# CobaltCrabby/ray_tracer

Measured on AMD Instinct MI355X. Metric: Mrays/s (reference-semantics closest-hit queries) at 1920x1080 Sponza, higher is better.
Workload: dtype f32; 1 GPU; sponza (synthetic-262267-tris), 1920x1080, 8 spp/step, bounceLimit 8, rows interleaved over 1 GPU(s), up to 10 steps in flight per rank (groups of 10+9+9+9); scene=sponza, assets=synthetic-262267-tris, width=1920, height=1080, frames_in_flight=10, pipeline=multi-kernel (k_trace_pw + k_shade per round)

## Files before the change

ray_tracer_amd/csrc/rt_device.hip:

```cpp

#include "rt_kernels.hip.h"
#include "bvh_build.hip.h"

#include <dlfcn.h>
#include <rccl/rccl.h>

#include <algorithm>
#include <chrono>
#include <cmath>
#include <cstdio>
#include <cstdlib>
#include <string>
#include <type_traits>
#include <vector>

namespace {

struct DevBuf {
    void* p = nullptr;
    size_t bytes = 0;
    DevBuf() = default;
    DevBuf(DevBuf&& o) noexcept : p(o.p), bytes(o.bytes) { o.p = nullptr; o.bytes = 0; }
    ~DevBuf() { release(); }
    void release() { if (p) (void)hipFree(p); p = nullptr; bytes = 0; }
};

struct EventPair { hipEvent_t a, b; };
#define RT_MAX_LANES 4
#define RT_FRAMES_MAX_SLOTS (24ull << 20)
struct RootInfo { uint32_t idx, cnt; float lo[3], hi[3]; uint32_t triFirst, triTotal; };
struct RowsOf {
    uint32_t width = 0, height = 0, row0 = 0, rowStride = 0, nRows = 0;
    bool whole(uint32_t w, uint32_t h) const { return width == w && height == h && row0 == 0 && rowStride == 1 && nRows == h; }
};

}

struct rt_ctx {
    std::string error;
    int device = 0, numCUs = 256;
    hipStream_t ownStream = nullptr, stream = nullptr;
    DevScene sc{};
    std::vector<DevBuf> sceneBufs;
    DevBuf texelBuf, texInfoBuf, triUVBuf, objTreeBuf, objCostBuf;
    DevBuf matBuf, sphereBuf, sphereMatBuf, objInvBuf, objFwdBuf, objMetaBuf, objBoxBuf, objSkipBuf, maskBoxBuf, emitBuf, emitPreBuf;
    std::vector<RayMaterial> hostMats;
    std::vector<uint32_t> hostSphereMat, hostObjMat, hostObjRoot, hostObjSampler;
    DevBuf objAlphaBuf;
    uint32_t maxLeafDepth = 0;
    std::vector<uint32_t> nodeRemap;
    std::vector<RootInfo> rootOf;
    bool cull = false;
    ncclComm_t comm = nullptr;
    int commRanks = 0, commRank = 0;
    DevBuf gatherBuf;
    DevBuf stateBuf, queueBuf, fbBuf, counterBuf, scratchBuf;
    DevBuf overflowBuf[RT_MAX_LANES];
    hipStream_t sideStream[RT_MAX_LANES - 1] = {};
    hipEvent_t forkEvent = nullptr, joinEvent[RT_MAX_LANES - 1] = {}, pollEventSide[RT_MAX_LANES - 1] = {};
    uint32_t capacity = 0;
    PathState ps{}; Queues q{};
    uint32_t* hostCounts = nullptr;
    uint32_t fbPixels = 0; bool fbValid = false;
    bool profiling = false;
    std::vector<EventPair> evPool;
    size_t evUsed = 0;
    hipEvent_t profBase = nullptr;
    DevCounters* snap = nullptr;
    hipEvent_t snapEvent = nullptr;
    hipEvent_t pollEvent = nullptr;
    DevBuf probeBuf;
    DevBuf waveTimeBuf;
    DevBuf aovBuf, aovCounterBuf;
    DevBuf shadeStatBuf;
    uint32_t aovPixels = 0; bool aovValid = false;
    RowsOf fbRows, aovRows;
    DevBuf dnWorkBuf, dnHostBuf, dnOutBuf;
    size_t dnOutPixels = 0; bool dnValid = false;

    struct Tuning {
        int objTreeMin = 48;
        int framesPerLaunch = 0;
        uint64_t framesMaxSlots = RT_FRAMES_MAX_SLOTS;
        int cameraReuse = 1;
        int lightQueries = 1;
        int lanes = 3;
        bool lanesSet = false;
        uint32_t lanesMinSlots = 1u << 20;
        int laneGridPct = 0;
        int traceVariant = 1;
        int pipeline = -1;
        uint32_t fusedBelowPixels = 4000000;
        uint32_t fusedBelowBoxTests = 70;
        int refill = 8;
        int refillMk = 16;
        bool refillMkSet = false;
        int chunk = 256;
        int ldsStackCap = 24;
        int fastLanes = 32;
        bool fastLanesSet = false;
        int wSetup = 16, wLeaf = 16;
        bool wSetupSet = false, wLeafSet = false;
        int wSetupFused = 16, wLeafFused = 24;
        int blocksPerCU = 0;
        int phaseStats = 0;
        int tileSlots = 1;
        int fastShare = 10;
        int maskIdentity = 0;
        int scatter = -1;
        int hotPairs = 2;
        int pixelRefill = 0;
        int batchPixels = 0;
        int batchFixed = 80;
        int fusedMaps = 0;
        int probe = 1;
    } tune;

    struct Measured {
        bool snapPending = false;
        unsigned long long snapBox = 0, snapRays = 0, snapSeg = 0, snapPaths = 0;
        double boxPerRay = -1.0;
        double segPerPath = -1.0;
    } meas;

    struct Reports {
        int lastPipeline = 0;
        int lastParts = 1;
        char lastKernel[96] = "";
        size_t waveTimesCount = 0;
        double traceMs = 0.0;
        uint64_t traceLaunches = 0;
        std::vector<std::pair<float, float>> traceSpans;
        uint64_t traceLaunchesTotal = 0, aovLaunches = 0;
        double bvhBuildMs = 0.0;
    } rep;
    int fail(const std::string& m) { error = m; return -1; }
    int hip(hipError_t e, const char* what) {
        if (e == hipSuccess) return 0;
        error = std::string(what) + ": " + hipGetErrorString(e);
        return -(int)e - 1000;
    }
};

#define RT_HIP(ctx, call)                                    \
    do {                                                     \
        int _rc = (ctx)->hip((call), #call);                 \
        if (_rc) return _rc;                                 \
    } while (0)

namespace {

int dev_alloc(rt_ctx* c, DevBuf& b, size_t bytes) {
    if (b.p && b.bytes >= bytes) return 0;
    b.release();
    if (bytes == 0) bytes = 256;
    RT_HIP(c, hipMalloc(&b.p, bytes));
    b.bytes = bytes;
    return 0;
}

int upload(rt_ctx* c, DevBuf& b, const void* src, size_t bytes) {
    int rc = dev_alloc(c, b, bytes);
    if (rc) return rc;
    if (bytes) RT_HIP(c, hipMemcpyAsync(b.p, src, bytes, hipMemcpyHostToDevice, c->stream));
    RT_HIP(c, hipStreamSynchronize(c->stream));
    return 0;
}

void pack_materials(const RayMaterial* m, uint32_t n, std::vector<float4>& out) {
    out.resize((size_t)std::max(n, 1u) * 3);
    for (uint32_t i = 0; i < n; i++) {
        out[3 * i + 0] = make_float4(m[i].albedo[0], m[i].albedo[1], m[i].albedo[2], m[i].reflectance);
// ... 793 lines not shown
    if ((rc = upload(c, c->sceneBufs[1], tpos.data(), tpos.size() * sizeof(float4)))) return rc;
    if ((rc = upload(c, c->sceneBufs[2], tnrm.data(), tnrm.size() * sizeof(float4)))) return rc;
    c->sc.nodes = (const float4*)c->sceneBufs[0].p;
    c->sc.triPos = (const float4*)c->sceneBufs[1].p;
    c->sc.triNrm = (const float4*)c->sceneBufs[2].p;
    if ((rc = upload(c, c->sceneBufs[3], leafFirst.data(), leafFirst.size() * 4))) return rc;
    c->sc.leafFirst = (const uint32_t*)c->sceneBufs[3].p;
    if ((rc = upload(c, c->sceneBufs[4], nodesPk.data(), nodesPk.size() * sizeof(float4)))) return rc;
    c->sc.nodesPk = (const float4*)c->sceneBufs[4].p;
    c->sc.nodeCount = devCount;
    c->sc.triCount = nTris;

    if (s->materialCount == 0) return c->fail("scene needs at least one material");
    if ((rc = rt_update_materials(c, s->materials, s->materialCount))) return rc;
    for (uint32_t i = 0; i < s->sphereCount; i++)
        if (s->spheres[i].materialIndex >= s->materialCount) return c->fail("sphere.materialIndex out of range");
    if ((rc = rt_update_spheres(c, s->spheres, s->sphereCount))) return rc;
    return rt_update_objects(c, s->objects, s->objectCount);
}

int rt_sync(rt_ctx* c) {
    if (!c) return -1;
    RT_HIP(c, hipStreamSynchronize(c->stream));
    return harvest_events(c);
}

}

namespace {
int check_tile(rt_ctx* c, const PushConstants* pc, uint32_t width, uint32_t height, uint32_t row0, uint32_t rowStride, uint32_t nRows,
               const char* fn) {
    if (width == 0 || height == 0 || rowStride == 0) return c->fail(std::string(fn) + ": bad image geometry");
    if (nRows && (uint64_t)row0 + (uint64_t)(nRows - 1) * rowStride >= height) return c->fail(std::string(fn) + ": rows exceed the image");
    if (!c->sc.nodes) return c->fail(std::string(fn) + " before rt_upload_scene");
    const RayTracerData& td = pc->rayTraceParams;
    if (td.sphereCount > c->sc.sphereCount) return c->fail("rayTraceParams.sphereCount exceeds the uploaded spheres");
    if (td.objectCount > c->sc.objectCount) return c->fail("rayTraceParams.objectCount exceeds the uploaded objects");
    return 0;
}

DevScene dispatch_scene(const rt_ctx* c, const RayTracerData& td) {
    DevScene sc = c->sc;
    sc.sphereCount = td.sphereCount;
    sc.objectCount = td.objectCount;
    if (sc.objectCount < c->sc.objectCount) { sc.reachCount = 0; sc.objTreeLevels = 0; }
    return sc;
}

FrameParams frame_camera(const rt_ctx* c, const PushConstants* pc, uint32_t width, uint32_t height, uint32_t row0, uint32_t rowStride,
                         uint32_t nRows, uint32_t nPixels) {
    FrameParams fp{};
    memcpy(fp.camRot, pc->camInfo.cameraRotation, 64);
    memcpy(fp.camPos, pc->camInfo.pos, 12);
    fp.planeHeight = pc->camInfo.nearPlane * rt_tan(rt_radians(pc->camInfo.fov * 0.5f)) * 2.f;
    fp.planeWidth = fp.planeHeight * pc->camInfo.aspectRatio;
    fp.bottomLeft[0] = -fp.planeWidth / 2.f;
    fp.bottomLeft[1] = -fp.planeHeight / 2.f;
    fp.bottomLeft[2] = 0.1f;
    fp.tiled = (c->tune.tileSlots && (width % 8u) == 0u) ? 1u : 0u;
    fp.width = width; fp.height = height; fp.row0 = row0; fp.rowStride = rowStride; fp.nRows = nRows; fp.nPixels = nPixels;
    return fp;
}

int choose_pipeline(const rt_ctx::Tuning& t, int pipeline, double boxPerRay, const DevScene& sc, uint32_t nSlots) {
    const bool shortRays = boxPerRay >= 0.0 && boxPerRay < (double)t.fusedBelowBoxTests;
    double sizeLimit = (double)t.fusedBelowPixels;
    if (boxPerRay > 90.0) sizeLimit = std::max(0.375 * sizeLimit, sizeLimit - (boxPerRay - 90.0) * (0.625 / 60.0) * sizeLimit);
    const bool bigScene = (uint64_t)sc.nodeCount * 32u + (uint64_t)sc.triCount * 48u > (4ull << 20);
    const bool shortButMissing = shortRays && bigScene && boxPerRay >= 25.0 && nSlots >= (10u << 20);
    const int chosen = pipeline >= 0 ? pipeline : (((double)nSlots < sizeLimit || (shortRays && !shortButMissing)) ? 1 : 0);
    return (sc.mapFlags && !t.fusedMaps) ? 0 : chosen;
}

int choose_parts(const rt_ctx::Tuning& t, const Dispatch& d, bool cull, double boxPerRay, uint32_t samples, uint32_t nSlots) {
    int nLanes = (samples > 0 && nSlots >= t.lanesMinSlots) ? std::max(1, std::min(t.lanes, (int)RT_MAX_LANES)) : 1;
    if (d.phaseStats) nLanes = 1;
    if (!t.lanesSet && cull && boxPerRay >= 150.0 && nSlots >= (8u << 20)) nLanes = 1;
    return nLanes;
}
int part_grid_pct(const rt_ctx::Tuning& t, int nLanes, uint32_t firstPartSlots) {
    return nLanes > 1 ? (t.laneGridPct > 0 ? t.laneGridPct : (firstPartSlots < 1200000u ? 40 : 50)) : 100;
}

int ensure_part_streams(rt_ctx* c, int nLanes) {
    for (int l = 1; l < nLanes; l++) {
        if (!c->sideStream[l - 1]) {
            if (hipStreamCreateWithFlags(&c->sideStream[l - 1], hipStreamNonBlocking) != hipSuccess) { c->sideStream[l - 1] = nullptr; nLanes = l; break; }
            if (hipEventCreateWithFlags(&c->joinEvent[l - 1], hipEventDisableTiming) != hipSuccess ||
                hipEventCreateWithFlags(&c->pollEventSide[l - 1], hipEventDisableTiming) != hipSuccess) { nLanes = l; break; }
        }
    }
    if (nLanes > 1 && !c->forkEvent && hipEventCreateWithFlags(&c->forkEvent, hipEventDisableTiming) != hipSuccess) { c->forkEvent = nullptr; nLanes = 1; }
    return nLanes;
}

struct Lane { Dispatch d; hipEvent_t poll; uint32_t begin, n, ubActive; int cur; bool pollPending, done; };
void slice_parts(rt_ctx* c, const Dispatch& d, uint32_t nSlots, uint32_t nFrames, int nLanes, Lane* lane) {
    const uint32_t unit = 256u * std::max(1u, nFrames);
    const uint32_t units = (nSlots + unit - 1) / unit;
    uint32_t at = 0;
    for (int l = 0; l < nLanes; l++) {
        const uint32_t u = units / (uint32_t)nLanes + ((uint32_t)l < units % (uint32_t)nLanes ? 1u : 0u);
        const uint32_t end = std::min(nSlots, at + u * unit);
        lane[l] = Lane{d, l ? c->pollEventSide[l - 1] : c->pollEvent, at, end - at, end - at, 0, false, end == at};
        lane[l].d.stream = l ? c->sideStream[l - 1] : c->stream; lane[l].d.counts = c->q.counts + 16 * l; lane[l].d.part = l;
        at = end;
    }
    const int gridPct = part_grid_pct(c->tune, nLanes, lane[0].n);
    for (int l = 0; l < nLanes; l++) lane[l].d.gridPct = gridPct;
}

int render_rounds(rt_ctx* c, const FrameParams& fp, Lane* lane, int nLanes) {
    DevCounters* dc = (DevCounters*)c->counterBuf.p;
    int rc = 0;
    if (nLanes > 1) {
        RT_HIP(c, hipEventRecord(c->forkEvent, c->stream));
        for (int l = 1; l < nLanes; l++) RT_HIP(c, hipStreamWaitEvent(lane[l].d.stream, c->forkEvent, 0));
    }
    const uint64_t maxRounds = (uint64_t)fp.samples * ((uint64_t)fp.bounceLimit + 1);
    for (uint64_t it = 0; it < maxRounds; it++) {
        bool any = false;
        for (int l = 0; l < nLanes; l++) {
            Lane& L = lane[l];
            if (L.done) continue;
            any = true;
            const hipStream_t stream = L.d.stream; uint32_t* const counts = L.d.counts;
            const int cur = L.cur, nxt = cur ^ 1;
            uint32_t* const active[2] = {c->q.active[0] + L.begin, c->q.active[1] + L.begin};
            uint32_t* const rays[2] = {c->q.rays[0] + 3 * (size_t)L.begin, c->q.rays[1] + 3 * (size_t)L.begin};
            hipLaunchKernelGGL(k_zero_counts, dim3(1), dim3(64), 0, stream, counts + nxt, counts + 2 + nxt, counts + 4, counts + 5 + nxt, counts + 7 + nxt);
            TraceArgs ta{rays[cur], counts + 2 + cur, nullptr, nullptr, dc, counts + 5 + cur, counts + 7 + cur, L.n};
            const uint64_t ubRays = std::min<uint64_t>((uint64_t)L.ubActive * 3, (uint64_t)L.n * 3);
            if ((rc = launch_trace(c, L.d, (uint32_t)ubRays, ta))) break;
            ShadeArgs sa{active[cur], counts + cur, active[nxt], rays[nxt], counts + nxt, counts + 2 + nxt, (ShadeStatStripe*)c->shadeStatBuf.p, counts + 5 + nxt, counts + 7 + nxt, L.n};
            if (L.d.sc.mapFlags & (RT_MAP_METALNESS | RT_MAP_BUMP)) hipLaunchKernelGGL(k_shade_maps, dim3((L.ubActive + RT_BLOCK - 1) / RT_BLOCK), dim3(RT_BLOCK), 0, stream, L.d.sc, c->ps, sa, fp);
            else hipLaunchKernelGGL(k_shade, dim3((L.ubActive + RT_BLOCK - 1) / RT_BLOCK), dim3(RT_BLOCK), 0, stream, L.d.sc, c->ps, sa, fp);
            L.cur = nxt;
            if (L.pollPending && hipEventQuery(L.poll) == hipSuccess) {
                L.pollPending = false;
                L.ubActive = std::min(L.ubActive, c->hostCounts[8 + l]);
                if (L.ubActive == 0) { L.done = true; continue; }
            }
            if (!L.pollPending && (it & 7u) == 7u) {
                if (hipMemcpyAsync(c->hostCounts + 8 + l, counts + L.cur, 4, hipMemcpyDeviceToHost, stream) == hipSuccess &&
                    hipEventRecord(L.poll, stream) == hipSuccess)
                    L.pollPending = true;
            }
        }
        if (!any || rc) break;
    }
    for (int l = 1; l < nLanes; l++) {
        RT_HIP(c, hipEventRecord(c->joinEvent[l - 1], lane[l].d.stream));
        RT_HIP(c, hipStreamWaitEvent(c->stream, c->joinEvent[l - 1], 0));
    }
    hipLaunchKernelGGL(k_fold_shade_stats, dim3(1), dim3(RT_STAT_STRIPES), 0, c->stream, (ShadeStatStripe*)c->shadeStatBuf.p, dc);
    return rc;
}

int render_parts(rt_ctx* c, const FrameParams& fp, const Dispatch& d, uint32_t nSlots, float4* fb) {
    const int nLanes = ensure_part_streams(c, choose_parts(c->tune, d, c->cull, c->meas.boxPerRay, fp.samples, nSlots));
    c->rep.lastParts = nLanes;
    Lane lane[RT_MAX_LANES];
    slice_parts(c, d, nSlots, fp.nFrames, nLanes, lane);
    for (int l = 0; l < nLanes; l++) {
        const Lane& L = lane[l];
        if (!L.n) continue;
        hipLaunchKernelGGL(k_raygen, dim3((L.n + RT_BLOCK - 1) / RT_BLOCK), dim3(RT_BLOCK), 0, c->stream, d.sc, c->ps,
                           c->q.active[0] + L.begin, c->q.rays[0] + 3 * (size_t)L.begin, fp, L.begin, L.begin + L.n);
        if (fp.samples > 0) hipLaunchKernelGGL(k_init_counts, dim3(1), dim3(64), 0, c->stream, L.d.counts, L.n);
    }
    RT_HIP(c, hipGetLastError());
    if (fp.samples > 0)
        if (int rc = render_rounds(c, fp, lane, nLanes)) return rc;
    const uint32_t blocksPix = (fp.nPixels + RT_BLOCK - 1) / RT_BLOCK;
    if (fp.nFrames > 1u) hipLaunchKernelGGL(k_blend_frames, dim3(blocksPix), dim3(RT_BLOCK), 0, c->stream, c->ps, fp, fb);
    else hipLaunchKernelGGL(k_resolve, dim3(blocksPix), dim3(RT_BLOCK), 0, c->stream, c->ps, fp, fb);
    RT_HIP(c, hipGetLastError());
    return 0;
}

int probe_ray_cost(rt_ctx* c, const FrameParams& fp, const Dispatch& d);

int render_dispatch(rt_ctx* c, const FrameParams& fp, const Dispatch& d, float4* fb) {
    const uint32_t nSlots = (uint32_t)dispatch_slots(fp.nPixels, fp.nFrames);
    int rc;
    poll_ray_cost(c);
    if (c->meas.boxPerRay < 0.0 && c->tune.probe && !d.probe && !d.sc.mapFlags && (uint64_t)fp.nPixels * fp.samples >= 8000000ull && fp.debug < 0 &&
        (rc = probe_ray_cost(c, fp, d)))
        return rc;
    const int pipeline = choose_pipeline(c->tune, d.pipeline, c->meas.boxPerRay, d.sc, nSlots);
    if (!d.probe) c->rep.lastPipeline = pipeline;
    if (pipeline == 1) {
        rc = launch_fused(c, d, fp, fb);
        if (!rc && fp.nFrames > 1u) {
            hipLaunchKernelGGL(k_blend_frames, dim3((fp.nPixels + RT_BLOCK - 1) / RT_BLOCK), dim3(RT_BLOCK), 0, c->stream, c->ps, fp, fb);
            rc = c->hip(hipGetLastError(), "k_blend_frames");
        }
    } else {
        rc = render_parts(c, fp, d, nSlots, fb);
    }
    if (!rc) request_ray_cost(c);
    return rc;
}

int probe_ray_cost(rt_ctx* c, const FrameParams& fp, const Dispatch& d) {
    const uint32_t rows = std::min(fp.nRows, 8u), skip = fp.nRows / rows;
    FrameParams p = fp;
    p.samples = 1; p.progressive = 0; p.debug = -1; p.nFrames = 1;
    p.row0 = fp.row0 + (skip / 2u) * fp.rowStride; p.rowStride = fp.rowStride * skip; p.nRows = rows; p.nPixels = rows * fp.width;
    Dispatch pd = d;
    pd.probe = true; pd.pipeline = 1; pd.profiled = false; pd.phaseStats = 0; pd.launches = nullptr;
    int rc = dev_alloc(c, c->probeBuf, (size_t)rows * fp.width * sizeof(float4));
    if (rc) return rc;
    DevCounters before, after;
    RT_HIP(c, hipMemcpyAsync(&before, c->counterBuf.p, sizeof(DevCounters), hipMemcpyDeviceToHost, c->stream));
    RT_HIP(c, hipStreamSynchronize(c->stream));
    if ((rc = render_dispatch(c, p, pd, (float4*)c->probeBuf.p))) return rc;
    RT_HIP(c, hipMemcpyAsync(&after, c->counterBuf.p, sizeof(DevCounters), hipMemcpyDeviceToHost, c->stream));
    RT_HIP(c, hipStreamSynchronize(c->stream));
// ... 384 lines not shown
    RT_HIP(c, hipStreamSynchronize(c->stream));
    c->meas.snapPending = false;
    c->meas.snapBox = 0; c->meas.snapRays = 0; c->meas.snapSeg = 0; c->meas.snapPaths = 0;
    int rc = harvest_events(c);
    c->rep.traceMs = 0.0; c->rep.traceLaunches = 0; c->rep.traceLaunchesTotal = 0; c->rep.aovLaunches = 0;
    c->rep.traceSpans.clear();
    return rc;
}

int rt_set_profiling(rt_ctx* c, int on) {
    if (!c) return -1;
    RT_HIP(c, hipStreamSynchronize(c->stream));
    int rc = harvest_events(c);
    c->profiling = on != 0;
    if (on) {
        if (!c->profBase) RT_HIP(c, hipEventCreate(&c->profBase));
        RT_HIP(c, hipEventRecord(c->profBase, c->stream));
        c->rep.traceSpans.clear();
    }
    return rc;
}

int rt_get_trace_busy_ms(rt_ctx* c, double* ms) {
    if (!c || !ms) return -1;
    RT_HIP(c, hipStreamSynchronize(c->stream));
    int rc = harvest_events(c);
    std::vector<std::pair<float, float>> v = c->rep.traceSpans;
    std::sort(v.begin(), v.end());
    double busy = 0.0, end = -1e300;
    for (const auto& iv : v) {
        if ((double)iv.first > end) { busy += (double)iv.second - (double)iv.first; end = iv.second; }
        else if ((double)iv.second > end) { busy += (double)iv.second - end; end = iv.second; }
    }
    *ms = busy;
    return rc;
}

int rt_get_trace_time_ms(rt_ctx* c, double* ms, uint64_t* launches) {
    if (!c) return -1;
    RT_HIP(c, hipStreamSynchronize(c->stream));
    int rc = harvest_events(c);
    if (ms) *ms = c->rep.traceMs;
    if (launches) *launches = c->rep.traceLaunches;
    return rc;
}

const char* rt_last_kernel(const rt_ctx* c) { return c ? c->rep.lastKernel : ""; }
int rt_last_parts(const rt_ctx* c) { return c ? c->rep.lastParts : 0; }

int rt_set_tuning(rt_ctx* c, const char* key, int value) {
    if (!c || !key) return -1;
    std::string k(key);
    if (k == "pipeline") { if (value < -1 || value > 1) return c->fail("pipeline: -1 (auto), 0 or 1"); c->tune.pipeline = value; }
    else if (k == "probe") { c->tune.probe = value ? 1 : 0; }
    else if (k == "frames_max_mslots") { if (value < 1 || value > 1000) return c->fail("frames_max_mslots: 1..1000 (millions of paths per multi-frame dispatch)"); c->tune.framesMaxSlots = (uint64_t)value << 20; }
    else if (k == "frames_per_launch") { if (value < 0) return c->fail("frames_per_launch >= 0"); c->tune.framesPerLaunch = value; }
    else if (k == "camera_reuse") { c->tune.cameraReuse = value ? 1 : 0; }
    else if (k == "light_queries") { c->tune.lightQueries = value ? 1 : 0; int rc = rebuild_emitters(c); if (rc) return rc; }
    else if (k == "fused_below_box_tests") { if (value < 0) return c->fail("fused_below_box_tests >= 0"); c->tune.fusedBelowBoxTests = (uint32_t)value; }
    else if (k == "fused_below_pixels") { if (value < 0) return c->fail("fused_below_pixels >= 0"); c->tune.fusedBelowPixels = (uint32_t)value; }
    else if (k == "trace_variant") { if (value < 0 || value > 1) return c->fail("trace_variant: 0 or 1"); c->tune.traceVariant = value; }
    else if (k == "refill") { if (value < 1 || value > 64) return c->fail("refill: 1..64"); c->tune.refill = value; c->tune.refillMk = value; c->tune.refillMkSet = true; }
    else if (k == "hot_pairs") { if (value < 0 || value > 2) return c->fail("hot_pairs: 0, 1 (six work-groups per CU) or 2 (five)"); c->tune.hotPairs = value; }
    else if (k == "mk_refill") { if (value < 1 || value > 64) return c->fail("mk_refill: 1..64"); c->tune.refillMk = value; c->tune.refillMkSet = true; }
    else if (k == "lds_stack") { if (value != 8 && value != 16 && value != 24) return c->fail("lds_stack: 8, 16 or 24"); c->tune.ldsStackCap = value; }
    else if (k == "fast_lanes") { if (value < 0 || value > 65) return c->fail("fast_lanes: 1..65 (0: back to the defaults)"); c->tune.fastLanesSet = value != 0; c->tune.fastLanes = value ? value : 32; }
    else if (k == "chunk") { if (value < 1 || value > 4096) return c->fail("chunk: 1..4096"); c->tune.chunk = value; }
    else if (k == "w_setup") { if (value < 1 || value > 512) return c->fail("w_setup: 1..512"); c->tune.wSetup = value; c->tune.wSetupFused = value; c->tune.wSetupSet = true; }
    else if (k == "w_leaf") { if (value < 1 || value > 512) return c->fail("w_leaf: 1..512"); c->tune.wLeaf = value; c->tune.wLeafFused = value; c->tune.wLeafSet = true; }
    else if (k == "mk_w_setup") { if (value < 1 || value > 512) return c->fail("mk_w_setup: 1..512"); c->tune.wSetup = value; c->tune.wSetupSet = true; }
    else if (k == "mk_w_leaf") { if (value < 1 || value > 512) return c->fail("mk_w_leaf: 1..512"); c->tune.wLeaf = value; }
    else if (k == "tile_slots") { c->tune.tileSlots = value != 0; }
    else if (k == "mask_identity") { c->tune.maskIdentity = value != 0; }
    else if (k == "fast_share") { if (value < 0 || value > 16) return c->fail("fast_share: 0..16"); c->tune.fastShare = value; }
    else if (k == "scatter") { if (value != -1 && value != 0 && value != 1 && value != 2 && value != 4 && value != 8 && value != 16) return c->fail("scatter: -1 (auto), 0, 1, 2, 4, 8 or 16"); c->tune.scatter = value; }
    else if (k == "fused_maps") { if (value < 0 || value > 1) return c->fail("fused_maps: 0 (map scenes take the multi-kernel pipeline) or 1 (they choose as usual)"); c->tune.fusedMaps = value; }
    else if (k == "pixel_refill") { if (value < 0 || value > (int)RT_WAVE) return c->fail("pixel_refill must be 0 (by ray length) .. 64"); c->tune.pixelRefill = value; }
    else if (k == "batch_pixels") { if (value < 0 || value > (int)RT_WAVE) return c->fail("batch_pixels must be 0 (auto) .. 64"); c->tune.batchPixels = value; }
    else if (k == "batch_fixed") { if (value < 0 || value > 4096) return c->fail("batch_fixed out of range"); c->tune.batchFixed = value; }
    else if (k == "phase_stats") { if (value < 0) return c->fail("phase_stats >= 0"); c->tune.phaseStats = value; }
    else if (k == "object_tree_min") { if (value < 0) return c->fail("object_tree_min >= 0"); c->tune.objTreeMin = value; }
    else if (k == "lanes") { if (value < 0 || value > RT_MAX_LANES) return c->fail("lanes: 1..4 (parts of a multi-kernel dispatch, each on its own stream), 0 = automatic"); c->tune.lanes = value ? value : 3; c->tune.lanesSet = value != 0; }
    else if (k == "lane_grid_pct") { if (value != 0 && (value < 10 || value > 100)) return c->fail("lane_grid_pct: 0 (by size) or 10..100"); c->tune.laneGridPct = value; }
    else if (k == "lanes_min_kslots") { if (value < 0) return c->fail("lanes_min_kslots >= 0"); c->tune.lanesMinSlots = (uint32_t)value << 10; }
    else if (k == "blocks_per_cu") { if (value < 0 || value > 8) return c->fail("blocks_per_cu: 0..8"); c->tune.blocksPerCU = value; }
    else return c->fail("unknown tuning key " + k);
    return 0;
}

int rt_last_pipeline(const rt_ctx* c) { return c ? c->rep.lastPipeline : -1; }
double rt_ray_cost(const rt_ctx* c) { return c ? c->meas.boxPerRay : -1.0; }

int rt_bvh_build(rt_ctx* c, const TrianglePoint* points, uint32_t pointCount, Triangle* triangles, float* centroids, uint32_t count,
                 uint32_t triIndex0, uint32_t nodeBase, BVHNode* nodesOut, uint32_t nodeCapacity, uint32_t* nodeCountOut, uint32_t statsOut[3]) {
    if (!c || !points || !triangles || !centroids || !nodesOut || !nodeCountOut) return -1;
    if (count == 0) return c->fail("rt_bvh_build: a mesh with 0 triangles");
    if (nodeCapacity < 2u * count - 1u) return c->fail("rt_bvh_build: node capacity below 2 * count - 1");
    RT_HIP(c, hipSetDevice(c->device));
    const auto t0 = std::chrono::steady_clock::now();
    const bool dbg = getenv("RT_BVH_DEBUG") != nullptr;
    auto mark = [&](const char* what) { if (dbg) fprintf(stderr, "[rt_bvh_build] %-12s %8.2f ms\n", what, std::chrono::duration<double, std::milli>(std::chrono::steady_clock::now() - t0).count()); };
    std::vector<float> verts((size_t)count * 9);
    for (uint32_t i = 0; i < count; i++) {
        const uint32_t vi[3] = {triangles[i].v0, triangles[i].v1, triangles[i].v2};
        for (int k = 0; k < 3; k++) {
            if (vi[k] >= pointCount) return c->fail("rt_bvh_build: triangle point index out of range");
            memcpy(&verts[(size_t)i * 9 + 3 * k], points[vi[k]].position, 12);
        }
    }
    const size_t nNodesMax = 2 * (size_t)count - 1;
    DevBuf bVerts, bCent, bPerm, bTmp, bHole, bNodes, bList, bCtr, bWide;
    const uint32_t maxChunks = (count + RT_BVH_CHUNK - 1) / RT_BVH_CHUNK;
    int rc;
    if ((rc = upload(c, bVerts, verts.data(), verts.size() * 4)) || (rc = upload(c, bCent, centroids, (size_t)count * 12)) ||
        (rc = dev_alloc(c, bPerm, (size_t)count * 4)) || (rc = dev_alloc(c, bTmp, (size_t)count * 4)) || (rc = dev_alloc(c, bHole, (size_t)count * 4)) ||
        (rc = dev_alloc(c, bNodes, nNodesMax * sizeof(BNode))) || (rc = dev_alloc(c, bList, 2 * (size_t)(count + 1) * 4)) || (rc = dev_alloc(c, bCtr, 64)) ||
        (rc = dev_alloc(c, bWide, RT_BVH_WIDE_NODES * sizeof(WideAcc) + (size_t)RT_BVH_WIDE_NODES * maxChunks * 4)))
        return rc;
    mark("uploaded");
    BvhBuildArgs a{(const float*)bVerts.p, (const float*)bCent.p, (uint32_t*)bPerm.p, (uint32_t*)bTmp.p, (uint32_t*)bHole.p, (BNode*)bNodes.p, (uint32_t*)bCtr.p};
    uint32_t* lists[2] = {(uint32_t*)bList.p, (uint32_t*)bList.p + (count + 1)};
    uint32_t* nextCount = (uint32_t*)bCtr.p + 1;
    hipLaunchKernelGGL(k_bvh_root, dim3(1), dim3(RT_BVH_BLOCK), 0, c->stream, a, count);
    uint32_t zero = 0, nCur = 1;
    hipError_t e = hipMemcpyAsync(lists[0], &zero, 4, hipMemcpyHostToDevice, c->stream);
    int cur = 0;
    std::vector<uint32_t> levelStart{0u, 1u};
    for (uint32_t level = 0; e == hipSuccess && nCur && level <= 64; level++) {
        e = hipMemsetAsync(nextCount, 0, 4, c->stream);
        if (e != hipSuccess) break;
        if (nCur <= RT_BVH_WIDE_NODES && count >= 8192u) {
            const WideArgs w{a, lists[cur], (WideAcc*)bWide.p, (uint32_t*)((char*)bWide.p + RT_BVH_WIDE_NODES * sizeof(WideAcc)), maxChunks, lists[cur ^ 1], nextCount};
            const dim3 gc(maxChunks, nCur), gn(nCur);
            hipLaunchKernelGGL(w_init, gn, dim3(64), 0, c->stream, w);
            hipLaunchKernelGGL(w_minmax, gc, dim3(256), 0, c->stream, w);
            hipLaunchKernelGGL(w_bins, gc, dim3(256), 0, c->stream, w);
            hipLaunchKernelGGL(w_sweep, gn, dim3(64), 0, c->stream, w);
            hipLaunchKernelGGL(w_count, gc, dim3(256), 0, c->stream, w);
            hipLaunchKernelGGL(w_scan, gn, dim3(64), 0, c->stream, w);
            hipLaunchKernelGGL(w_left, gc, dim3(256), 0, c->stream, w);
            hipLaunchKernelGGL(w_right, gc, dim3(256), 0, c->stream, w);
            hipLaunchKernelGGL(w_commit, gc, dim3(256), 0, c->stream, w);
            hipLaunchKernelGGL(w_finish, gn, dim3(64), 0, c->stream, w);
        }
        else if (nCur <= 32) hipLaunchKernelGGL(k_bvh_level<1024>, dim3(nCur), dim3(1024), 0, c->stream, a, lists[cur], lists[cur ^ 1], nextCount);
        else if (count / nCur >= 128) hipLaunchKernelGGL(k_bvh_level<256>, dim3(nCur), dim3(256), 0, c->stream, a, lists[cur], lists[cur ^ 1], nextCount);
        else hipLaunchKernelGGL(k_bvh_level<64>, dim3(nCur), dim3(64), 0, c->stream, a, lists[cur], lists[cur ^ 1], nextCount);
        e = hipMemcpyAsync(&nCur, nextCount, 4, hipMemcpyDeviceToHost, c->stream);
        if (e == hipSuccess) e = hipStreamSynchronize(c->stream);
        if (nCur) levelStart.push_back(levelStart.back() + nCur);
        cur ^= 1;
    }
    if (e == hipSuccess) e = hipGetLastError();
    mark("levels done");
    uint32_t nNodes = 0;
    if (e == hipSuccess) e = hipMemcpy(&nNodes, bCtr.p, 4, hipMemcpyDeviceToHost);
    if (e == hipSuccess && (nNodes == 0 || nNodes > nNodesMax || nNodes != levelStart.back())) return c->fail("rt_bvh_build: node counter out of range");

    DevBuf bNum, bOut;
    uint32_t hstats[3] = {0u, 0xffffffffu, 0u};
    if (e == hipSuccess && ((rc = dev_alloc(c, bNum, 3 * (size_t)nNodes * 4 + 64)) || (rc = dev_alloc(c, bOut, (size_t)nNodes * sizeof(BVHNode)))))
        return rc;
    std::vector<uint32_t> perm(count);
    if (e == hipSuccess) {
        uint32_t* nb = (uint32_t*)bNum.p;
        uint32_t* dstats = nb + 3 * (size_t)nNodes;
// ... 260 lines not shown
```

ray_tracer_amd/csrc/rt_kernels.hip.h:

```cpp
#pragma once

#include <hip/hip_runtime.h>
#include <stdint.h>

#include "rt_amd.h"
#include "rt_det_math.h"
#include "rt_probe.h"

#define RT_WAVE 64
#ifndef RT_TE_REG
#define RT_MAP_METALNESS 1u
#define RT_MAP_ALPHA 2u
#define RT_MAP_BUMP 4u
#ifndef RT_QUEUE_ORDER
#define RT_QUEUE_ORDER 0
#endif
#define RT_TE_REG 1
#endif
#ifndef RT_OBJTREE
#define RT_OBJTREE 1
#endif
#ifndef RT_SHADE_IDENT
#define RT_SHADE_IDENT 1
#endif
// ... 1231 lines not shown
                float invP = 1.f / rrProb;
                att = rt_scale(att, invP);
                ro = rt_add(hit.hitPoint, rt_scale(rt_scale(hit.normal, originSign), 0.00001f));
                rd = sampledDir;
                j++;
                if (j > fp.bounceLimit) done = true;
                else wantAux = diffuse;
            }
        }
    } else {
        total = rt_add(total, rt_mul(att, environment_light(fp.env, rd)));
        done = true;
    }

    if (done) {
        nPaths = 1;
        float4 acc = ps.accum()[slot];
        if (zeroed) total = rt_v3(0.f, 0.f, 0.f);
        const rt_vec3 sum = rt_add(f4xyz(acc), total);
        ps.accum()[slot] = mk4(sum, 0.f);
        samplesDone++;
        if (samplesDone < fp.samples) {
            ro = rt_v3(fp.camPos[0], fp.camPos[1], fp.camPos[2]);
            rd = f4xyz(ps.camDir()[slot]);
            att = rt_v3(1.f, 1.f, 1.f);
            total = rt_v3(0.f, 0.f, 0.f);
            specular = false;
            misW = 1.f;
            j = 0;
            alive = true;
            wantAux = false;
        }
    } else {
        alive = true;
    }

    if (alive) {
        if (done && fp.camReuse) {
            if (!QUEUED) ps.hit(RAY_MAIN)[slot] = ps.camHit()[slot];
            auxMask |= 4u;
        } else {
            const float4 seed = sphere_seed(sc, ro, rd, withMask);
            if (QUEUED && seed_is_blank(seed)) auxMask |= 8u;
            else ps.hit(RAY_MAIN)[slot] = seed;
        }
        if (wantAux) {
            float4 sL = sphere_seed(sc, auxOrigin, auxL, withMask), sC = sphere_seed(sc, auxOrigin, auxC, withMask);
            auxMask |= 3u;
            if (sc.emitMode) {
                float tL, tC;
                emitter_min_t2(sc, auxOrigin, auxL, auxC, tL, tC, emitTests);
                if (!(tL < RT_MISS_DST) || sL.x < tL) { sL.x = RT_MISS_DST; sL.y = __uint_as_float(RT_HIT_NONE); auxMask &= ~1u; }
                else sL.w = tL;
                if (!(tC < RT_MISS_DST) || sC.x < tC) { sC.x = RT_MISS_DST; sC.y = __uint_as_float(RT_HIT_NONE); auxMask &= ~2u; }
                else sC.w = tC;
            }
            const bool albedoFinite = !(rt_isnan(auxAlbedo.x) || rt_isnan(auxAlbedo.y) || rt_isnan(auxAlbedo.z) || rt_isinf(auxAlbedo.x) || rt_isinf(auxAlbedo.y) || rt_isinf(auxAlbedo.z));
            if ((auxMask & 3u) == 0u && albedoFinite) {
                float m2 = auxCosPdfC * auxCosPdfC / (0.f * 0.f + auxCosPdfC * auxCosPdfC);
                if (rt_isnan(m2)) m2 = 0.f;
                misW = m2;
                wantAux = false;
            } else {
                if (auxMask & 1u) ps.hit(RAY_NEE)[slot] = sL;
                if (auxMask & 2u) ps.hit(RAY_PROBE)[slot] = sC;
                if (auxMask & 3u) ps.auxO()[slot] = mk4(auxOrigin, 0.f);
                if (auxMask & 1u) ps.auxDL()[slot] = mk4(auxL, 0.f);
                if (auxMask & 2u) ps.auxDC()[slot] = mk4(auxC, 0.f);
                ps.pendAlbedo()[slot] = mk4(auxAlbedo, auxNdotL);
                ps.pendMis()[slot] = make_float4(auxCosL, auxCosC, auxCosPdfL, auxCosPdfC);
            }
        }
        const uint32_t answered = wantAux ? (((auxMask & 1u) ? 0u : 0x20000000u) | ((auxMask & 2u) ? 0u : 0x10000000u)) : 0u;
        ps.rayO()[slot] = mk4(ro, misW);
        ps.rayD()[slot] = mk4u(rd, state);
        ps.att()[slot] = mk4u(att, j | (wantAux ? 0x80000000u : 0u) | (specular ? 0x40000000u : 0u) | answered);
        const float4 nT = mk4u(total, samplesDone);
        if (!QUEUED || __float_as_uint(nT.x) != __float_as_uint(sT.x) || __float_as_uint(nT.y) != __float_as_uint(sT.y) ||
            __float_as_uint(nT.z) != __float_as_uint(sT.z) || __float_as_uint(nT.w) != __float_as_uint(sT.w))
            ps.total()[slot] = nT;
    }
}

template <bool MAPS>
__device__ __forceinline__ void shade_block(const DevScene& sc, const PathState& ps, const ShadeArgs& sa, const FrameParams& fp) {
    __shared__ uint32_t s_cnt[RT_BLOCK / RT_WAVE][8];
    __shared__ uint32_t s_base[4];
    const uint32_t n = *sa.inCount;
    if (blockIdx.x * RT_BLOCK >= n) return;
    const uint32_t gid = blockIdx.x * RT_BLOCK + threadIdx.x;
    const bool live = gid < n;

    bool alive = false;
    uint32_t auxMask = 0;
    uint32_t slot = 0;
    uint32_t refRays = 0, nPaths = 0, emitTests = 0;
    bool path = live;
    if (live) {
        slot = sa.inActive[gid];
        path = slot != 0xffffffffu;
        if (path) shade_path<MAPS, true>(sc, ps, fp, slot, alive, auxMask, refRays, nPaths, emitTests);
    }

    const unsigned long long mAlive = __ballot(alive), mM = __ballot(alive && !(auxMask & 4u));
    const unsigned long long mL = __ballot(alive && (auxMask & 1u)), mC = __ballot(alive && (auxMask & 2u));
    const uint32_t nAlive = __popcll(mAlive), nM = __popcll(mM), nL = __popcll(mL), nC = __popcll(mC);
    const uint32_t wRef = wave_sum_u32(refRays), wPaths = wave_sum_u32(nPaths), wSeg = wave_sum_u32(path ? 1u : 0u), wEmit = wave_sum_u32(emitTests);
    const uint32_t wv = threadIdx.x / RT_WAVE;
    if (lane_id() == 0) {
        s_cnt[wv][0] = nAlive; s_cnt[wv][1] = nM; s_cnt[wv][2] = wRef; s_cnt[wv][3] = wPaths; s_cnt[wv][4] = wSeg; s_cnt[wv][5] = wEmit; s_cnt[wv][6] = nL; s_cnt[wv][7] = nC;
    }
    __syncthreads();
    if (threadIdx.x == 0) {
        uint32_t tA = 0, tR = 0, tRef = 0, tP = 0, tS = 0, tE = 0, tX = 0, tY = 0;
        for (int w = 0; w < RT_BLOCK / RT_WAVE; w++) { tA += s_cnt[w][0]; tR += s_cnt[w][1]; tRef += s_cnt[w][2]; tP += s_cnt[w][3]; tS += s_cnt[w][4]; tE += s_cnt[w][5]; tX += s_cnt[w][6]; tY += s_cnt[w][7]; }
        s_base[0] = tA ? atomicAdd(sa.outActiveCount, tA) : 0u;
        s_base[1] = tR ? atomicAdd(sa.outRayCount, tR) : 0u;
        s_base[2] = tX ? atomicAdd(RT_QUEUE_ORDER ? sa.outAuxCount2 : sa.outAuxCount, tX) : 0u;
        s_base[3] = tY ? atomicAdd(RT_QUEUE_ORDER ? sa.outAuxCount : sa.outAuxCount2, tY) : 0u;
        ShadeStatStripe* const st = sa.stats + (blockIdx.x & (RT_STAT_STRIPES - 1u));
        atomicAdd(&st->raysReference, (unsigned long long)tRef);
        if (tP) atomicAdd(&st->paths, (unsigned long long)tP);
        atomicAdd(&st->segments, (unsigned long long)tS);
        if (tE) atomicAdd(&st->emitterTests, (unsigned long long)tE);
    }
    __syncthreads();
    if (alive) {
        uint32_t baseA = s_base[0], baseR = s_base[1];
        uint32_t baseX = (RT_QUEUE_ORDER ? 2u : 1u) * sa.auxOffset + s_base[2], baseY = (RT_QUEUE_ORDER ? 1u : 2u) * sa.auxOffset + s_base[3];
        for (uint32_t w = 0; w < wv; w++) { baseA += s_cnt[w][0]; baseR += s_cnt[w][1]; baseX += s_cnt[w][6]; baseY += s_cnt[w][7]; }
        sa.outActive[baseA + lanes_below(mAlive)] = slot;
        if (!(auxMask & 4u)) sa.outRays[baseR + lanes_below(mM)] = (slot << 2) | ((auxMask & 8u) ? RAY_MAIN_BLANK : (uint32_t)RAY_MAIN);
        if (auxMask & 1u) sa.outRays[baseX + lanes_below(mL)] = (slot << 2) | RAY_NEE;
        if (auxMask & 2u) sa.outRays[baseY + lanes_below(mC)] = (slot << 2) | RAY_PROBE;
    }
}

__global__ __launch_bounds__(RT_BLOCK) void k_shade(DevScene sc, PathState ps, ShadeArgs sa, FrameParams fp) { shade_block<false>(sc, ps, sa, fp); }
__global__ __launch_bounds__(RT_BLOCK) void k_shade_maps(DevScene sc, PathState ps, ShadeArgs sa, FrameParams fp) { shade_block<true>(sc, ps, sa, fp); }

__device__ __forceinline__ rt_vec3 blend_frame(const FrameParams& fp, uint32_t frameCount, float4 oldc, float4 accum) {
    rt_vec3 out = f4xyz(accum);
    float fs = (float)fp.samples;
    out = rt_v3(out.x / fs, out.y / fs, out.z / fs);
    float weight = 1.f / ((float)frameCount + 1.f);
    rt_vec3 blended = rt_add(rt_scale(rt_v3(oldc.x, oldc.y, oldc.z), 1.f - weight), rt_scale(out, weight));
    rt_vec3 fin = fp.progressive ? blended : out;
    if (rt_isnan(fin.x) || rt_isnan(fin.y) || rt_isnan(fin.z) || rt_isinf(fin.x) || rt_isinf(fin.y) || rt_isinf(fin.z))
        fin = rt_v3(1.f, 0.f, 1.f);
    return fin;
}

__device__ __forceinline__ void resolve_pixel(const PathState& ps, const FrameParams& fp, float4* rgba, uint32_t slot) {
    uint32_t gx, gy, krow;
    slot_to_pixel(fp, slot, gx, gy, krow);
    const size_t px = (size_t)krow * fp.width + gx;
    rt_vec3 fin = blend_frame(fp, fp.frameCount, rgba[px], ps.accum()[slot]);
    float s0 = (float)ps.statBox()[slot], s1 = (float)ps.statTri()[slot];
    float boxCap = (float)fp.boxCap, triCap = (float)fp.triCap;
    if (fp.debug == 0) {
        fin = s0 > boxCap ? rt_v3(1.f, 0.f, 0.f) : rt_v3(s0 / boxCap, s0 / boxCap, s0 / boxCap);
    } else if (fp.debug == 1) {
        fin = s1 > triCap ? rt_v3(1.f, 0.f, 0.f) : rt_v3(s1 / triCap, s1 / triCap, s1 / triCap);
    } else if (fp.debug == 2) {
        fin = rt_v3(s0 / boxCap, 0.f, s1 / triCap);
    }
    rgba[px] = make_float4(fin.x, fin.y, fin.z, 1.f);
}

__global__ __launch_bounds__(RT_BLOCK) void k_blend_frames(PathState ps, FrameParams fp, float4* rgba) {
    const uint32_t slot = blockIdx.x * RT_BLOCK + threadIdx.x;
    if (slot >= fp.nPixels) return;
    uint32_t gx, gy, krow;
    slot_to_pixel(fp, frame_slot(fp, 0u, slot), gx, gy, krow);
    const size_t px = (size_t)krow * fp.width + gx;
    float4 c = rgba[px];
    for (uint32_t f = 0; f < fp.nFrames; f++) {
        const rt_vec3 fin = blend_frame(fp, fp.frameCount + f, c, ps.accum()[frame_slot(fp, f, slot)]);
        c = make_float4(fin.x, fin.y, fin.z, 1.f);
    }
    rgba[px] = c;
}

__global__ __launch_bounds__(RT_BLOCK) void k_resolve(PathState ps, FrameParams fp, float4* rgba) {
    uint32_t slot = blockIdx.x * RT_BLOCK + threadIdx.x;
    if (slot >= fp.nPixels) return;
    resolve_pixel(ps, fp, rgba, slot);
}

struct FusedArgs {
    uint32_t* batchHead;
    float4* rgba;
    DevCounters* counters;
    uint32_t* overflow;
    uint32_t refill, wSetup, wLeaf, fastLanes;
    uint32_t batchPixels;
    uint32_t scatter;
    uint32_t fastShare;
    unsigned long long* waveTimes;
    uint32_t pixelRefill;
};

template <typename T>
__device__ __forceinline__ const T* opaque_kernarg() {
    unsigned long long v = (unsigned long long)__builtin_amdgcn_kernarg_segment_ptr();
    asm volatile("" : "+s"(v));
    return (const T*)(const RT_AS_CONSTANT T*)v;
}

struct FusedKernArgs {
    DevScene sc;
    PathState ps;
    FrameParams fp;
    FusedArgs fa;
};

template <int STACK, bool OVF, bool PIX, bool CULL>
__global__ __launch_bounds__(RT_BLOCK, 5) void k_render_fused(FusedKernArgs ka) {
    constexpr bool ALPHA = false, MAPS = false;
#include "rt_fused_body.hip.inc"
}
template <bool PIX>
__global__ __launch_bounds__(RT_BLOCK, RT_FUSED_MAPS_BLOCKS) void k_render_fused_maps(FusedKernArgs ka) {
    constexpr int STACK = 24;
    constexpr bool OVF = true, CULL = true, ALPHA = true, MAPS = true;
#include "rt_fused_body.hip.inc"
}

__global__ __launch_bounds__(RT_BLOCK) void k_hit_details(DevScene sc, PathState ps, uint32_t n, const uint32_t* perRayBox,
                                                          const uint32_t* perRayTri, RtHit* out) {
    uint32_t i = blockIdx.x * RT_BLOCK + threadIdx.x;
    if (i >= n) return;
    RtHit h;
    memset(&h, 0, sizeof(h));
    const float4 hm = ps.hit(RAY_MAIN)[i];
    h.dst = hm.x;
    uint32_t obj = __float_as_uint(hm.y);
    const uint32_t tri = __float_as_uint(hm.z);
    h.boxTests = perRayBox[i];
    h.triTests = perRayTri[i];
    if (obj != RT_HIT_NONE) {
        FullHit f = reconstruct_hit<true>(sc, f4xyz(ps.rayO()[i]), f4xyz(ps.rayD()[i]), obj, tri);
        h.didHit = 1;
        h.isSphere = (obj & RT_HIT_SPHERE) ? 1u : 0u;
        h.objectHitIndex = obj & ~RT_HIT_SPHERE;
        h.triHitIndex = h.isSphere ? 0u : tri;
        h.materialIndex = f.materialIndex;
        h.frontFace = f.frontFace;
        h.hitPoint[0] = f.hitPoint.x; h.hitPoint[1] = f.hitPoint.y; h.hitPoint[2] = f.hitPoint.z;
        h.normal[0] = f.normal.x; h.normal[1] = f.normal.y; h.normal[2] = f.normal.z;
    }
    out[i] = h;
}

__global__ __launch_bounds__(RT_BLOCK) void k_seed_rays(DevScene sc, PathState ps, uint32_t n) {
    uint32_t i = blockIdx.x * RT_BLOCK + threadIdx.x;
    if (i < n) ps.hit(RAY_MAIN)[i] = sphere_seed(sc, f4xyz(ps.rayO()[i]), f4xyz(ps.rayD()[i]));
}

struct AovOut { float4 *normalDepth, *position, *albedo, *rayDir; uint4* ids; };

__global__ __launch_bounds__(RT_BLOCK) void k_aov_rays(DevScene sc, PathState ps, FrameParams fp) {
    const uint32_t slot = blockIdx.x * RT_BLOCK + threadIdx.x;
    if (slot >= fp.nPixels) return;
    uint32_t gx, gy, krow;
    slot_to_pixel(fp, slot, gx, gy, krow);
    const rt_vec3 ro = rt_v3(fp.camPos[0], fp.camPos[1], fp.camPos[2]), rd = primary_dir(fp, gx, gy);
    ps.rayO()[slot] = mk4(ro, 0.f);
    ps.rayD()[slot] = mk4(rd, 0.f);
    ps.hit(RAY_MAIN)[slot] = sphere_seed(sc, ro, rd);
}

__global__ __launch_bounds__(RT_BLOCK) void k_aov_resolve(DevScene sc, PathState ps, FrameParams fp, AovOut out) {
    const uint32_t slot = blockIdx.x * RT_BLOCK + threadIdx.x;
    if (slot >= fp.nPixels) return;
    uint32_t gx, gy, krow;
    slot_to_pixel(fp, slot, gx, gy, krow);
    const size_t px = (size_t)krow * fp.width + gx;
    const rt_vec3 ro = f4xyz(ps.rayO()[slot]), rd = f4xyz(ps.rayD()[slot]);
    const float4 hm = ps.hit(RAY_MAIN)[slot];
    const uint32_t obj = __float_as_uint(hm.y), tri = __float_as_uint(hm.z);
    float4 normalDepth = make_float4(0.f, 0.f, 0.f, hm.x), position = make_float4(0.f, 0.f, 0.f, 0.f), albedo = position;
    uint4 ids = make_uint4(RT_HIT_NONE, RT_HIT_NONE, RT_HIT_NONE, 0u);
    if (obj != RT_HIT_NONE) {
        const bool sphere = (obj & RT_HIT_SPHERE) != 0u;
        const FullHit f = reconstruct_hit<true>(sc, ro, rd, obj, tri);
        const float4* mp = rt_global(sc.mats) + 3 * f.materialIndex;
        const float4 mA = mp[0];
        rt_vec3 a = rt_v3(mA.x, mA.y, mA.z);
        const uint32_t texSlot = __float_as_uint(mp[2].y);
        if (texSlot < sc.texCount && !sphere) a = rt_mul(a, albedo_texel(sc, texSlot, tri, obj, ro, rd));
// ... 200 lines not shown
```

Baseline: 4735 Mrays/s.

## Shade several block-sized chunks per block with one batched atomic reservation

The shade kernel is templated on a group count G, so each block processes up to G chunks of RT_BLOCK paths. It stashes per-chunk slot and aux bits in LDS, then does one block-wide prefix and one set of queue atomics for all chunks. The host picks G automatically so the grid keeps at least 4096 blocks. The kernel also reads its arguments through an opaque kernarg pointer to limit SGPR pressure, and pins waves_per_eu to 4. This is meant to cut global atomic traffic and per-block overhead, at the cost of more LDS use, a serial loop over chunks within each block, and a fixed occupancy hint.

```diff
diff --git a/ray_tracer_amd/csrc/rt_device.hip b/ray_tracer_amd/csrc/rt_device.hip
--- a/ray_tracer_amd/csrc/rt_device.hip
+++ b/ray_tracer_amd/csrc/rt_device.hip
@@ -88,6 +88,7 @@
         bool lanesSet = false;
         uint32_t lanesMinSlots = 1u << 20;
         int laneGridPct = 0;
+        int shadeGroup = 0;
         int traceVariant = 1;
         int pipeline = -1;
         uint32_t fusedBelowPixels = 4000000;
@@ -1047,6 +1048,28 @@
     return nLanes > 1 ? (t.laneGridPct > 0 ? t.laneGridPct : (firstPartSlots < 1200000u ? 40 : 50)) : 100;
 }
 
+#define RT_SHADE_MIN_GROUPS 4096u
+int shade_group_for(const rt_ctx::Tuning& t, uint32_t ubActive) {
+    if (t.shadeGroup > 0) return t.shadeGroup;
+    int g = 8;
+    while (g > 1 && (ubActive + (uint32_t)g * RT_BLOCK - 1u) / ((uint32_t)g * RT_BLOCK) < RT_SHADE_MIN_GROUPS) g >>= 1;
+    return g;
+}
+template <int G>
+void launch_shade_g(const DevScene& sc, const PathState& ps, const ShadeArgs& sa, const FrameParams& fp, uint32_t ubActive, hipStream_t stream) {
+    const dim3 grid((ubActive + G * RT_BLOCK - 1u) / (G * RT_BLOCK));
+    if (sc.mapFlags & (RT_MAP_METALNESS | RT_MAP_BUMP)) hipLaunchKernelGGL(k_shade_maps<G>, grid, dim3(RT_BLOCK), 0, stream, sc, ps, sa, fp);
+    else hipLaunchKernelGGL(k_shade<G>, grid, dim3(RT_BLOCK), 0, stream, sc, ps, sa, fp);
+}
+void launch_shade(const rt_ctx::Tuning& t, const DevScene& sc, const PathState& ps, const ShadeArgs& sa, const FrameParams& fp, uint32_t ubActive, hipStream_t stream) {
+    switch (shade_group_for(t, ubActive)) {
+        case 8: launch_shade_g<8>(sc, ps, sa, fp, ubActive, stream); break;
+        case 4: launch_shade_g<4>(sc, ps, sa, fp, ubActive, stream); break;
+        case 2: launch_shade_g<2>(sc, ps, sa, fp, ubActive, stream); break;
+        default: launch_shade_g<1>(sc, ps, sa, fp, ubActive, stream); break;
+    }
+}
+
 int ensure_part_streams(rt_ctx* c, int nLanes) {
     for (int l = 1; l < nLanes; l++) {
         if (!c->sideStream[l - 1]) {
@@ -1098,8 +1121,7 @@
             const uint64_t ubRays = std::min<uint64_t>((uint64_t)L.ubActive * 3, (uint64_t)L.n * 3);
             if ((rc = launch_trace(c, L.d, (uint32_t)ubRays, ta))) break;
             ShadeArgs sa{active[cur], counts + cur, active[nxt], rays[nxt], counts + nxt, counts + 2 + nxt, (ShadeStatStripe*)c->shadeStatBuf.p, counts + 5 + nxt, counts + 7 + nxt, L.n};
-            if (L.d.sc.mapFlags & (RT_MAP_METALNESS | RT_MAP_BUMP)) hipLaunchKernelGGL(k_shade_maps, dim3((L.ubActive + RT_BLOCK - 1) / RT_BLOCK), dim3(RT_BLOCK), 0, stream, L.d.sc, c->ps, sa, fp);
-            else hipLaunchKernelGGL(k_shade, dim3((L.ubActive + RT_BLOCK - 1) / RT_BLOCK), dim3(RT_BLOCK), 0, stream, L.d.sc, c->ps, sa, fp);
+            launch_shade(c->tune, L.d.sc, c->ps, sa, fp, L.ubActive, stream);
             L.cur = nxt;
             if (L.pollPending && hipEventQuery(L.poll) == hipSuccess) {
                 L.pollPending = false;
@@ -1650,6 +1672,7 @@
     else if (k == "object_tree_min") { if (value < 0) return c->fail("object_tree_min >= 0"); c->tune.objTreeMin = value; }
     else if (k == "lanes") { if (value < 0 || value > RT_MAX_LANES) return c->fail("lanes: 1..4 (parts of a multi-kernel dispatch, each on its own stream), 0 = automatic"); c->tune.lanes = value ? value : 3; c->tune.lanesSet = value != 0; }
     else if (k == "lane_grid_pct") { if (value != 0 && (value < 10 || value > 100)) return c->fail("lane_grid_pct: 0 (by size) or 10..100"); c->tune.laneGridPct = value; }
+    else if (k == "shade_group") { if (value != 0 && value != 1 && value != 2 && value != 4 && value != 8) return c->fail("shade_group: 0 (by the launch's size), 1, 2, 4 or 8"); c->tune.shadeGroup = value; }
     else if (k == "lanes_min_kslots") { if (value < 0) return c->fail("lanes_min_kslots >= 0"); c->tune.lanesMinSlots = (uint32_t)value << 10; }
     else if (k == "blocks_per_cu") { if (value < 0 || value > 8) return c->fail("blocks_per_cu: 0..8"); c->tune.blocksPerCU = value; }
     else return c->fail("unknown tuning key " + k);
diff --git a/ray_tracer_amd/csrc/rt_kernels.hip.h b/ray_tracer_amd/csrc/rt_kernels.hip.h
--- a/ray_tracer_amd/csrc/rt_kernels.hip.h
+++ b/ray_tracer_amd/csrc/rt_kernels.hip.h
@@ -1337,62 +1337,95 @@
     }
 }
 
-template <bool MAPS>
+template <typename T>
+__device__ __forceinline__ const T* opaque_kernarg() {
+    unsigned long long v = (unsigned long long)__builtin_amdgcn_kernarg_segment_ptr();
+    asm volatile("" : "+s"(v));
+    return (const T*)(const RT_AS_CONSTANT T*)v;
+}
+
+struct ShadeKernArgs { DevScene sc; PathState ps; ShadeArgs sa; FrameParams fp; };
+static_assert(offsetof(ShadeKernArgs, ps) == sizeof(DevScene) && offsetof(ShadeKernArgs, sa) == sizeof(DevScene) + sizeof(PathState) &&
+              offsetof(ShadeKernArgs, fp) == sizeof(DevScene) + sizeof(PathState) + sizeof(ShadeArgs), "k_shade's arguments lie without padding");
+
+template <bool MAPS, int G>
 __device__ __forceinline__ void shade_block(const DevScene& sc, const PathState& ps, const ShadeArgs& sa, const FrameParams& fp) {
-    __shared__ uint32_t s_cnt[RT_BLOCK / RT_WAVE][8];
-    __shared__ uint32_t s_base[4];
+    constexpr int WAVES = RT_BLOCK / RT_WAVE;
+    __shared__ uint32_t s_cnt[G * WAVES][8];
+    __shared__ uint32_t s_slot[G > 1 ? G : 1][G > 1 ? RT_BLOCK : 1];
+    __shared__ uint8_t s_bits[G > 1 ? G : 1][G > 1 ? RT_BLOCK : 1];
+    __shared__ uint32_t s_base[8];
     const uint32_t n = *sa.inCount;
-    if (blockIdx.x * RT_BLOCK >= n) return;
-    const uint32_t gid = blockIdx.x * RT_BLOCK + threadIdx.x;
-    const bool live = gid < n;
+    const uint32_t first = blockIdx.x * (uint32_t)(G * RT_BLOCK);
+    if (first >= n) return;
+    const uint32_t nChunks = G > 1 ? min((uint32_t)G, (n - first + RT_BLOCK - 1u) / RT_BLOCK) : 1u;
+    const uint32_t wv = threadIdx.x / RT_WAVE;
 
     bool alive = false;
     uint32_t auxMask = 0;
     uint32_t slot = 0;
-    uint32_t refRays = 0, nPaths = 0, emitTests = 0;
-    bool path = live;
-    if (live) {
-        slot = sa.inActive[gid];
-        path = slot != 0xffffffffu;
-        if (path) shade_path<MAPS, true>(sc, ps, fp, slot, alive, auxMask, refRays, nPaths, emitTests);
-    }
-
-    const unsigned long long mAlive = __ballot(alive), mM = __ballot(alive && !(auxMask & 4u));
-    const unsigned long long mL = __ballot(alive && (auxMask & 1u)), mC = __ballot(alive && (auxMask & 2u));
-    const uint32_t nAlive = __popcll(mAlive), nM = __popcll(mM), nL = __popcll(mL), nC = __popcll(mC);
-    const uint32_t wRef = wave_sum_u32(refRays), wPaths = wave_sum_u32(nPaths), wSeg = wave_sum_u32(path ? 1u : 0u), wEmit = wave_sum_u32(emitTests);
-    const uint32_t wv = threadIdx.x / RT_WAVE;
-    if (lane_id() == 0) {
-        s_cnt[wv][0] = nAlive; s_cnt[wv][1] = nM; s_cnt[wv][2] = wRef; s_cnt[wv][3] = wPaths; s_cnt[wv][4] = wSeg; s_cnt[wv][5] = wEmit; s_cnt[wv][6] = nL; s_cnt[wv][7] = nC;
+#pragma unroll 1
+    for (uint32_t g = 0; g < nChunks; g++) {
+        const DevScene* sq = &sc; const PathState* pq = &ps; const FrameParams* fq = &fp; const ShadeArgs* aq = &sa;
+        if (G > 1) { const ShadeKernArgs* kq = opaque_kernarg<ShadeKernArgs>(); sq = &kq->sc; pq = &kq->ps; fq = &kq->fp; aq = &kq->sa; }
+        const uint32_t gid = first + g * RT_BLOCK + threadIdx.x;
+        const bool live = gid < n;
+        alive = false; auxMask = 0; slot = 0;
+        uint32_t refRays = 0, nPaths = 0, emitTests = 0;
+        bool path = live;
+        if (live) {
+            slot = aq->inActive[gid];
+            path = slot != 0xffffffffu;
+            if (path) shade_path<MAPS, true>(*sq, *pq, *fq, slot, alive, auxMask, refRays, nPaths, emitTests);
+        }
+        const uint32_t nAlive = __popcll(__ballot(alive)), nM = __popcll(__ballot(alive && !(auxMask & 4u)));
+        const uint32_t nL = __popcll(__ballot(alive && (auxMask & 1u))), nC = __popcll(__ballot(alive && (auxMask & 2u)));
+        const uint32_t wRef = wave_sum_u32(refRays), wPaths = wave_sum_u32(nPaths), wSeg = wave_sum_u32(path ? 1u : 0u), wEmit = wave_sum_u32(emitTests);
+        if (lane_id() == 0) {
+            uint32_t* const cw = s_cnt[g * WAVES + wv];
+            cw[0] = nAlive; cw[1] = nM; cw[2] = wRef; cw[3] = wPaths; cw[4] = wSeg; cw[5] = wEmit; cw[6] = nL; cw[7] = nC;
+        }
+        if (G > 1) { s_slot[g][threadIdx.x] = slot; s_bits[g][threadIdx.x] = (uint8_t)(auxMask | (alive ? 16u : 0u)); }
     }
     __syncthreads();
-    if (threadIdx.x == 0) {
-        uint32_t tA = 0, tR = 0, tRef = 0, tP = 0, tS = 0, tE = 0, tX = 0, tY = 0;
-        for (int w = 0; w < RT_BLOCK / RT_WAVE; w++) { tA += s_cnt[w][0]; tR += s_cnt[w][1]; tRef += s_cnt[w][2]; tP += s_cnt[w][3]; tS += s_cnt[w][4]; tE += s_cnt[w][5]; tX += s_cnt[w][6]; tY += s_cnt[w][7]; }
-        s_base[0] = tA ? atomicAdd(sa.outActiveCount, tA) : 0u;
-        s_base[1] = tR ? atomicAdd(sa.outRayCount, tR) : 0u;
-        s_base[2] = tX ? atomicAdd(RT_QUEUE_ORDER ? sa.outAuxCount2 : sa.outAuxCount, tX) : 0u;
-        s_base[3] = tY ? atomicAdd(RT_QUEUE_ORDER ? sa.outAuxCount : sa.outAuxCount2, tY) : 0u;
-        ShadeStatStripe* const st = sa.stats + (blockIdx.x & (RT_STAT_STRIPES - 1u));
-        atomicAdd(&st->raysReference, (unsigned long long)tRef);
-        if (tP) atomicAdd(&st->paths, (unsigned long long)tP);
-        atomicAdd(&st->segments, (unsigned long long)tS);
-        if (tE) atomicAdd(&st->emitterTests, (unsigned long long)tE);
+    const ShadeArgs* ra = &sa;
+    if (G > 1) ra = &opaque_kernarg<ShadeKernArgs>()->sa;
+    if (threadIdx.x < 8u) {
+        const uint32_t k = threadIdx.x;
+        uint32_t run = 0;
+        for (uint32_t i = 0; i < nChunks * WAVES; i++) { const uint32_t v = s_cnt[i][k]; s_cnt[i][k] = run; run += v; }
+        uint32_t at = 0;
+        if (k == 0u && run) at = atomicAdd(ra->outActiveCount, run);
+        if (k == 1u && run) at = atomicAdd(ra->outRayCount, run);
+        if (k == 6u && run) at = atomicAdd(RT_QUEUE_ORDER ? ra->outAuxCount2 : ra->outAuxCount, run);
+        if (k == 7u && run) at = atomicAdd(RT_QUEUE_ORDER ? ra->outAuxCount : ra->outAuxCount2, run);
+        if (k >= 2u && k < 6u && run)
+            atomicAdd(&(ra->stats + (blockIdx.x & (RT_STAT_STRIPES - 1u)))->raysReference + (k - 2u), (unsigned long long)run);
+        s_base[k] = at;
     }
     __syncthreads();
-    if (alive) {
-        uint32_t baseA = s_base[0], baseR = s_base[1];
-        uint32_t baseX = (RT_QUEUE_ORDER ? 2u : 1u) * sa.auxOffset + s_base[2], baseY = (RT_QUEUE_ORDER ? 1u : 2u) * sa.auxOffset + s_base[3];
-        for (uint32_t w = 0; w < wv; w++) { baseA += s_cnt[w][0]; baseR += s_cnt[w][1]; baseX += s_cnt[w][6]; baseY += s_cnt[w][7]; }
-        sa.outActive[baseA + lanes_below(mAlive)] = slot;
-        if (!(auxMask & 4u)) sa.outRays[baseR + lanes_below(mM)] = (slot << 2) | ((auxMask & 8u) ? RAY_MAIN_BLANK : (uint32_t)RAY_MAIN);
-        if (auxMask & 1u) sa.outRays[baseX + lanes_below(mL)] = (slot << 2) | RAY_NEE;
-        if (auxMask & 2u) sa.outRays[baseY + lanes_below(mC)] = (slot << 2) | RAY_PROBE;
-    }
-}
-
-__global__ __launch_bounds__(RT_BLOCK) void k_shade(DevScene sc, PathState ps, ShadeArgs sa, FrameParams fp) { shade_block<false>(sc, ps, sa, fp); }
-__global__ __launch_bounds__(RT_BLOCK) void k_shade_maps(DevScene sc, PathState ps, ShadeArgs sa, FrameParams fp) { shade_block<true>(sc, ps, sa, fp); }
+    const uint32_t baseA = s_base[0], baseR = s_base[1];
+    const uint32_t baseX = (RT_QUEUE_ORDER ? 2u : 1u) * ra->auxOffset + s_base[6], baseY = (RT_QUEUE_ORDER ? 1u : 2u) * ra->auxOffset + s_base[7];
+#pragma unroll 1
+    for (uint32_t g = 0; g < nChunks; g++) {
+        if (G > 1) { slot = s_slot[g][threadIdx.x]; const uint32_t b = s_bits[g][threadIdx.x]; auxMask = b & 15u; alive = (b & 16u) != 0u; }
+        const unsigned long long mAlive = __ballot(alive), mM = __ballot(alive && !(auxMask & 4u));
+        const unsigned long long mL = __ballot(alive && (auxMask & 1u)), mC = __ballot(alive && (auxMask & 2u));
+        if (alive) {
+            const uint32_t* const cw = s_cnt[g * WAVES + wv];
+            ra->outActive[baseA + cw[0] + lanes_below(mAlive)] = slot;
+            if (!(auxMask & 4u)) ra->outRays[baseR + cw[1] + lanes_below(mM)] = (slot << 2) | ((auxMask & 8u) ? RAY_MAIN_BLANK : (uint32_t)RAY_MAIN);
+            if (auxMask & 1u) ra->outRays[baseX + cw[6] + lanes_below(mL)] = (slot << 2) | RAY_NEE;
+            if (auxMask & 2u) ra->outRays[baseY + cw[7] + lanes_below(mC)] = (slot << 2) | RAY_PROBE;
+        }
+    }
+}
+
+#define RT_SHADE_WAVES __attribute__((amdgpu_waves_per_eu(4, 4)))
+template <int G>
+__global__ __launch_bounds__(RT_BLOCK) RT_SHADE_WAVES void k_shade(DevScene sc, PathState ps, ShadeArgs sa, FrameParams fp) { shade_block<false, G>(sc, ps, sa, fp); }
+template <int G>
+__global__ __launch_bounds__(RT_BLOCK) RT_SHADE_WAVES void k_shade_maps(DevScene sc, PathState ps, ShadeArgs sa, FrameParams fp) { shade_block<true, G>(sc, ps, sa, fp); }
 
 __device__ __forceinline__ rt_vec3 blend_frame(const FrameParams& fp, uint32_t frameCount, float4 oldc, float4 accum) {
     rt_vec3 out = f4xyz(accum);
@@ -1455,13 +1488,6 @@
     unsigned long long* waveTimes;
     uint32_t pixelRefill;
 };
-
-template <typename T>
-__device__ __forceinline__ const T* opaque_kernarg() {
-    unsigned long long v = (unsigned long long)__builtin_amdgcn_kernarg_segment_ptr();
-    asm volatile("" : "+s"(v));
-    return (const T*)(const RT_AS_CONSTANT T*)v;
-}
 
 struct FusedKernArgs {
     DevScene sc;
```

New measurement: 4574 Mrays/s. -3.4%, worse.
